# diharaw/hybrid-rendering

Hardware: AMD Instinct MI355X
Metric: shadow Mrays/s over the fully denoised frame (1 spp trace + SVGF temporal + 4x a-trous) (higher is better)
Workload: dtype f32; 1 GPU; 1920x1080 procedural Sponza-like (277968 tris) ray-traced shadows 1spp + SVGF denoise; trace_launch_order=heaviest tiles of the last frame first (csrc/tile_order.h), rays_per_frame_per_gpu=729543, pixels_per_gpu=2073600, bvh_nodes=23425

## Files before the change

hybrid_rendering_amd/api.py:

```python
from __future__ import annotations

import ctypes as C
import os

import numpy as np

_HERE = os.path.dirname(os.path.abspath(__file__))
LIB_PATH = os.environ.get("HR_LIBRARY") or os.path.join(_HERE, "libhybrid_rendering_amd.so")



class hr_light(C.Structure):
    _fields_ = [("data0", C.c_float * 4), ("data1", C.c_float * 4), ("data2", C.c_float * 4), ("data3", C.c_float * 4)]


class hr_ubo(C.Structure):
    _fields_ = [("view_inverse", C.c_float * 16), ("proj_inverse", C.c_float * 16), ("view_proj_inverse", C.c_float * 16),
                ("prev_view_proj", C.c_float * 16), ("view_proj", C.c_float * 16), ("cam_pos", C.c_float * 4),
                ("current_prev_jitter", C.c_float * 4), ("light", hr_light)]


assert C.sizeof(hr_ubo) == 416


# ... 28 lines not shown


class hr_band(C.Structure):
    _fields_ = [("band_y0", C.c_int32), ("band_y1", C.c_int32), ("halo", C.c_int32), ("history_halo", C.c_int32)]


HR_MAX_STAGES = 16


class hr_stage_times(C.Structure):
    _fields_ = [("n_stages", C.c_int32), ("name", C.c_char_p * HR_MAX_STAGES), ("ms", C.c_float * HR_MAX_STAGES), ("bytes", C.c_uint64 * HR_MAX_STAGES)]


class hr_shadows_params(C.Structure):
    _fields_ = [("denoise", C.c_int32), ("bias", C.c_float), ("alpha", C.c_float), ("moments_alpha", C.c_float), ("phi_visibility", C.c_float),
                ("phi_normal", C.c_float), ("sigma_depth", C.c_float), ("power", C.c_float), ("radius", C.c_int32),
                ("filter_iterations", C.c_int32), ("feedback_iteration", C.c_int32), ("exact", C.c_int32)]


class hr_ao_params(C.Structure):
    _fields_ = [("denoise", C.c_int32), ("ray_length", C.c_float), ("bias", C.c_float), ("alpha", C.c_float), ("blur_radius", C.c_int32),
                ("power", C.c_float), ("spp", C.c_int32), ("exact", C.c_int32)]


HR_FORMAT = {1: ("R32_UINT", 4), 2: ("R16F", 2), 3: ("RG16F", 4), 4: ("RGBA16F", 8), 5: ("R32F", 4), 6: ("RGBA8", 4), 0: ("R8", 1)}
OUTPUT_RAY_TRACE, OUTPUT_TEMPORAL_ACCUMULATION, OUTPUT_ATROUS, OUTPUT_UPSAMPLE = 0, 1, 2, 3
SCALE_FULL_RES, SCALE_HALF_RES, SCALE_QUARTER_RES = 0, 1, 2

ABI_SYMBOLS = [
    "hr_status_string", "hr_last_error", "hr_version", "hr_api_revision", "hr_ctx_create", "hr_ctx_destroy", "hr_ctx_device", "hr_scene_create", "hr_scene_get_info", "hr_scene_id", "hr_scene_create_instanced", "hr_scene_update_instances", "hr_scene_instance_count", "hr_scene_rebuild_top_level", "hr_scene_top_level_rebuilds", "hr_scene_read_bvh", "hr_set_markers", "hr_markers_log",
    "hr_scene_destroy", "hr_trace_any_hit", "hr_trace_closest_hit", "hr_gbuffer_raycast", "hr_shadows_default_params", "hr_shadows_create",
    "hr_shadows_render", "hr_shadows_output", "hr_shadows_reset_history", "hr_shadows_destroy", "hr_shadows_ray_trace", "hr_shadows_denoise", "hr_shadows_temporal",
    "hr_shadows_atrous_iteration", "hr_shadows_upsample", "hr_shadows_image", "hr_shadows_history_apron_exceeded", "hr_shadows_set_profiling", "hr_shadows_get_stage_times",
    "hr_gbuffer_mip_nearest", "hr_bvh_build_info", "hr_bvh_selfcheck", "hr_shadows_ray_count", "hr_shadows_tile_ray_counts", "hr_shadows_trace_stats", "hr_shadows_trace_stats_timed", "hr_shadows_launch_order", "hr_shadows_trace_divergence", "hr_selftest_math",
]

_lib = None


class HRError(RuntimeError):
    pass


def lib():
    global _lib
    if _lib is None:
        if not os.path.exists(LIB_PATH):
            raise HRError(f"{LIB_PATH} not built: run `python -m hybrid_rendering_amd.build` (hipcc, gfx950). No CPU fallback exists.")
        try:
            import torch
        except Exception:
            pass
        _lib = C.CDLL(LIB_PATH)
        _lib.hr_status_string.restype = C.c_char_p
        _lib.hr_last_error.restype = C.c_char_p
        _lib.hr_version.restype = C.c_char_p
        _lib.hr_scene_id.restype = C.c_uint64
        _lib.hr_scene_id.argtypes = [C.c_void_p]
    return _lib


def _check(status: int, what: str):
    if status != 0:
        L = lib()
        raise HRError(f"{what}: {L.hr_status_string(status).decode()} — {L.hr_last_error().decode()}")


# ... 368 lines not shown
```

hybrid_rendering_amd/csrc/device_math.h:

```cpp
#pragma once
#include <hip/hip_runtime.h>
#include <stdint.h>

#define HR_DEV __device__ __forceinline__

namespace hr {

struct f3 { float x, y, z; };

HR_DEV float hr_sqrt(float x) { return __builtin_sqrtf(x); }
HR_DEV f3 mk3(float x, float y, float z) { f3 r; r.x = x; r.y = y; r.z = z; return r; }
HR_DEV f3 add3(f3 a, f3 b) { return mk3(a.x + b.x, a.y + b.y, a.z + b.z); }
HR_DEV f3 sub3(f3 a, f3 b) { return mk3(a.x - b.x, a.y - b.y, a.z - b.z); }
HR_DEV f3 scale3(f3 a, float s) { return mk3(a.x * s, a.y * s, a.z * s); }
HR_DEV f3 neg3(f3 a) { return mk3(-a.x, -a.y, -a.z); }
HR_DEV float dot3(f3 a, f3 b) { return (a.x * b.x + a.y * b.y) + a.z * b.z; }
HR_DEV f3 cross3(f3 a, f3 b) { return mk3(a.y * b.z - b.y * a.z, a.z * b.x - b.z * a.x, a.x * b.y - b.x * a.y); }
HR_DEV float len3(f3 a) { return hr_sqrt(dot3(a, a)); }
HR_DEV f3 normalize3(f3 a)
{
    float inv = __fdiv_rn(1.0f, hr_sqrt(dot3(a, a)));
    return scale3(a, inv);
}
HR_DEV float min2(float a, float b) { return a < b ? a : b; }
// ... 65 lines not shown
};
HR_DEV DivBy div_prepare(float d)
{
    DivBy D;
    D.d = d;
    const float r0 = __builtin_amdgcn_rcpf(d);
    const float e0 = hr_fma(-d, r0, 1.0f);
    D.r1   = hr_fma(e0, r0, r0);
    D.fast = d >= 1e-6f && d <= 1e6f;
    return D;
}
HR_DEV float div_by(float n, const DivBy& D)
{
    const float an = fabsf(n);
    if (D.fast && (n == 0.0f || (an >= 1e-12f && an <= 3e5f)))
    {
        const float q0 = n * D.r1;
        const float e1 = hr_fma(-D.d, q0, n);
        const float q1 = hr_fma(e1, D.r1, q0);
        const float e2 = hr_fma(-D.d, q1, n);
        return hr_fma(e2, D.r1, q1);
    }
    return __fdiv_rn(n, D.d);
}
HR_DEV float div_by_inrange(float n, const DivBy& D)
{
    const float q0 = n * D.r1;
    const float e1 = hr_fma(-D.d, q0, n);
    const float q1 = hr_fma(e1, D.r1, q0);
    const float e2 = hr_fma(-D.d, q1, n);
    return hr_fma(e2, D.r1, q1);
}
HR_DEV float div_by_if(bool inrange, float n, const DivBy& D) { return inrange ? div_by_inrange(n, D) : __fdiv_rn(n, D.d); }

HR_DEV float det_log(float x)
{
    if (x <= 0.0f) return -1.0e30f;
    uint32_t u = __float_as_uint(x);
    int      e = (int)(u >> 23) - 126;
    float    m = __uint_as_float((u & 0x007fffffu) | 0x3f000000u);
    if (m < 0.707106781186547524f)
    {
        e -= 1;
        m = m + m - 1.0f;
    }
    else
        m = m - 1.0f;
    float z  = m * m;
    float y  = ((((((((7.0376836292e-2f * m - 1.1514610310e-1f) * m + 1.1676998740e-1f) * m - 1.2420140846e-1f) * m + 1.4249322787e-1f) * m - 1.6668057665e-1f) * m + 2.0000714765e-1f) * m - 2.4999993993e-1f) * m + 3.3333331174e-1f) * m * z;
    float fe = (float)e;
    y        = y + fe * -2.12194440e-4f;
    y        = y - 0.5f * z;
    float r  = m + y;
    r        = r + fe * 0.693359375f;
    return r;
}

HR_DEV float det_pow(float x, float y)
{
    if (x <= 0.0f) return 0.0f;
    return det_exp(y * det_log(x));
}

HR_DEV float det_powi(float x, int n)
{
    float r = 1.0f, b = x;
// ... 23 lines not shown
        float nx = (1.0f - fabsf(v.y)) * (step1(0.0f, v.x) * 2.0f - 1.0f);
        float ny = (1.0f - fabsf(v.x)) * (step1(0.0f, v.y) * 2.0f - 1.0f);
        v.x = nx;
        v.y = ny;
    }
    return normalize3(v);
}

HR_DEV void oct_encode(f3 n, float& ox, float& oy)
{
    float inv = __fdiv_rn(1.0f, (fabsf(n.x) + fabsf(n.y)) + fabsf(n.z));
    float px = n.x * inv, py = n.y * inv;
    if (n.z > 0.0f) { ox = px; oy = py; }
    else
    {
        ox = (1.0f - fabsf(py)) * (step1(0.0f, px) * 2.0f - 1.0f);
        oy = (1.0f - fabsf(px)) * (step1(0.0f, py) * 2.0f - 1.0f);
    }
}

HR_DEV int trace_lane_kind(int x, int y, int w, int h, int y0, int y1)
{
    const int gy = (y >> 2) << 2;
    if (gy >= h) return 0;
    if (y < h) return (y < y0 || y >= y1) ? 0 : (x < w ? 1 : 2);
    return (gy >= y0 && gy < y1) ? 2 : 0;
}

HR_DEV f3 world_pos_from_depth(float u, float v, float ndc_depth, const float* __restrict__ view_proj_inverse)
{
    f4 wp = mul_m4(view_proj_inverse, u * 2.0f - 1.0f, v * 2.0f - 1.0f, ndc_depth, 1.0f);
    return mk3(__fdiv_rn(wp.x, wp.w), __fdiv_rn(wp.y, wp.w), __fdiv_rn(wp.z, wp.w));
}

HR_DEV float luminance(f3 rgb) { return max2(dot3(rgb, mk3(0.299f, 0.587f, 0.114f)), 0.0001f); }

HR_DEV uint32_t blue_noise_texel(int cx, int cy, const uint8_t* __restrict__ sr) { return *(const uint32_t*)(sr + (((cy & 127) * 128 + (cx & 127)) << 2)); }
HR_DEV float sample_blue_noise_t(uint32_t t, int sample_index, int dim, const uint8_t* __restrict__ sobol)
{
    sample_index &= 255;
    dim &= 3;
    int ranked = sample_index ^ (int)((t >> 16) & 0xffu);
    int value  = (int)sobol[ranked * 4 + dim];
    value ^= (int)((t >> ((dim & 1) * 8)) & 0xffu);
    return (0.5f + (float)value) * 0.00390625f;
}
HR_DEV float sample_blue_noise(int cx, int cy, int sample_index, int dim, const uint8_t* __restrict__ sobol, const uint8_t* __restrict__ sr)
{
    return sample_blue_noise_t(blue_noise_texel(cx, cy, sr), sample_index, dim, sobol);
}

}
```

hybrid_rendering_amd/csrc/shading.h:

```cpp
#pragma once
#include "../../include/hr_api.h"
#include "traverse.h"

#ifdef HR_PROBE_FAST_HIT
namespace hr { HR_DEV f3 probe_normalize3(f3 a) { return scale3(a, __builtin_amdgcn_rsqf(dot3(a, a))); } }
#define __fdiv_rn(a, b) ((a) * __builtin_amdgcn_rcpf(b))
#define hr_sqrt(x) __builtin_amdgcn_sqrtf(x)
#define normalize3(v) probe_normalize3(v)
#endif

namespace hr {

#define HR_EPSILON 0.0001f

struct Rng { uint32_t x, y; };
HR_DEV uint32_t rng_rotl(uint32_t x, uint32_t k) { return (x << k) | (x >> (32 - k)); }
HR_DEV uint32_t rng_next(Rng& r)
{
    uint32_t result = r.x * 0x9e3779bbu;
    r.y ^= r.x;
    r.x = rng_rotl(r.x, 26) ^ r.y ^ (r.y << 9);
    r.y = rng_rotl(r.y, 13);
    return result;
}
// ... 475 lines not shown
            {
                const float* qt = s.tangents + q * 9;
                tg = add3(add3(scale3(mk3(qt[0], qt[1], qt[2]), b0), scale3(mk3(qt[3], qt[4], qt[5]), b1)), scale3(mk3(qt[6], qt[7], qt[8]), b2));
            }
            tg = ir ? normalize3(inst_mul3(ir->m, normalize3(tg))) : normalize3(normalize3(tg));
            const f3 T = normalize3(tg), Nn = normalize3(o.N);
            sample_texture(s, mt[1], tu, tv, c);
            const f3 tn = normalize3(sub3(scale3(mk3(c[0], c[1], c[2]), 2.0f), one3()));
            o.N = normalize3(add3(add3(scale3(T, tn.x), scale3(T, tn.y)), scale3(Nn, tn.z)));
        }
    }
    return o;
}

HR_DEV void fetch_light_hard(const hr_light& L, f3 Wo, f3 P, f3 N, f3& Li, f3& Wi, f3& Wh, float& t_max, float& attenuation)
{
    const int type = (int)L.data3[0];
    const f3  ldir = mk3(L.data0[0], L.data0[1], L.data0[2]);
    Li = scale3(mk3(L.data2[0], L.data2[1], L.data2[2]), L.data0[3]);
    if (type == 0) { Wi = ldir; t_max = 10000.0f; attenuation = 1.0f; }
    else
    {
        const f3 to_light = sub3(mk3(L.data1[0], L.data1[1], L.data1[2]), P);
        Wi                = normalize3(to_light);
        const float dist  = len3(to_light);
        t_max             = dist;
        if (type == 1) attenuation = __fdiv_rn(1.0f, dist * dist);
        else attenuation = __fdiv_rn(smoothstep1(L.data3[1], L.data3[2], dot3(Wi, ldir)), dist * dist);
    }
    Wh          = normalize3(add3(Wo, Wi));
    attenuation = attenuation * clamp1(dot3(N, Wi), 0.0f, 1.0f);
}

HR_DEV void fetch_light_shadow(const hr_light& L, f3 P, f3 N, float rx, float ry, f3& Wi, float& t_max, float& attenuation)
{
    const int type = (int)L.data3[0];
    const f3  ldir = mk3(L.data0[0], L.data0[1], L.data0[2]);
    f3        light_dir;
    float     radius;
    if (type == 0)
    {
        light_dir   = ldir;
        radius      = L.data1[3];
        t_max       = 10000.0f;
        attenuation = 1.0f;
    }
    else
    {
        f3    to_light = sub3(mk3(L.data1[0], L.data1[1], L.data1[2]), P);
        light_dir      = normalize3(to_light);
        float dist     = len3(to_light);
        radius         = __fdiv_rn(L.data1[3], dist);
        t_max          = dist;
        attenuation    = __fdiv_rn(1.0f, dist * dist);
    }
    f3    tangent   = normalize3(cross3(light_dir, mk3(0.0f, 1.0f, 0.0f)));
    f3    bitangent = normalize3(cross3(tangent, light_dir));
    float pr        = radius * hr_sqrt(rx);
    float pa        = ry * 2.0f * HR_M_PI;
    float s, c;
    det_sincos(pa, s, c);
    float dx = pr * c, dy = pr * s;
    Wi       = normalize3(add3(add3(light_dir, scale3(tangent, dx)), scale3(bitangent, dy)));
    if (type == 2)
    {
        float aa    = smoothstep1(L.data3[1], L.data3[2], dot3(Wi, ldir));
        attenuation = __fdiv_rn(aa, t_max * t_max);
    }
    attenuation = attenuation * clamp1(dot3(N, Wi), 0.0f, 1.0f);
}

struct TraceCtx
{
    const Node8*  nodes;
    const TriGPU* tris;
    uint32_t*     wave_stack;
    int           lane;
    DivCounters*  dv = nullptr;
    uint32_t      nn = 0, nt = 0;
};

template <bool STATS = false>
HR_DEV f3 direct_lighting(TraceCtx& tc, const hr_light& light, f3 Wo, f3 N, f3 P, f3 F0, f3 diffuse_color, float roughness, f3 T,
                          bool sample_sky, float r2x, float r2y, const CubeMap& sky, uint32_t& rays)
{
    f3       Lo = mk3(0.0f, 0.0f, 0.0f);
    const f3 ray_origin = add3(P, scale3(N, 0.1f));
    uint32_t nn = 0, nt = 0;
    {
        f3    Li, Wi, Wh;
        float t_max, attenuation;
        fetch_light_hard(light, Wo, P, N, Li, Wi, Wh, t_max, attenuation);
#ifndef HR_ABL_NO_SECONDARY
        if (attenuation > 0.0f)
        {
            rays++;
            attenuation = attenuation * (trace_any<STATS>(tc.nodes, tc.tris, ray_origin, Wi, 0.01f, t_max, tc.wave_stack, tc.lane, nn, nt, 0u, tc.dv) ? 0.0f : 1.0f);
        }
#endif
        const f3 brdf = evaluate_uber_brdf(diffuse_color, roughness, N, F0, Wo, Wh, Wi);
        Lo = add3(Lo, mul3(scale3(mul3(T, brdf), attenuation), Li));
    }
// ... 62 lines not shown
```

hybrid_rendering_amd/csrc/shadows.hip:

```cpp
#include "hr_internal.h"
#include "reproject.h"
#include "traverse.h"
#include "shading.h"
#include "upsample.h"
#include "pass_args.h"
#include "tile_order.h"

using namespace hr;

struct TraceArgs
{
    float           vpi[16];
    hr_light        light;
    const float*    depth;
    const uint2*    gb2;
    const uint8_t*  sobol;
    const uint8_t*  sr;
    uint32_t*       mask;
    uint16_t*       ray_slots;
    const Node8*    nodes;
    const TriGPU*   tris;
    unsigned long long* stats;
    unsigned long long* timeline;
    int             w, h;
    int             y0, y1;
    int             mw;
    int             tiles_x, tiles_y, tile_y0, debug_skip_traversal, debug_only_tx, debug_only_ty;
    float           bias;
    uint32_t        num_frames;
    uint32_t*       occluder;
    uint32_t        n_tri_refs;
    const uint32_t* order;
    uint16_t*       cost;
};

#define TRACE_WAVES 1
#ifndef SHADOWS_TRACE_EU
#define SHADOWS_TRACE_EU 1
#endif
template <bool STATS>
__global__ __launch_bounds__(64 * TRACE_WAVES, SHADOWS_TRACE_EU) void k_shadows_trace(TraceArgs a)
{
    __shared__ uint32_t s_stack[TRACE_WAVES][HR_STACK_ENTRIES * 64];
    const int lane = threadIdx.x & 63, wave = threadIdx.x >> 6;
    const int launch_slot = blockIdx.x * TRACE_WAVES + wave;
    if (launch_slot >= a.tiles_x * a.tiles_y) return;
    const int slot = a.order ? (int)a.order[launch_slot] : launch_slot;
    const int tx = slot % a.tiles_x, ty_local = slot / a.tiles_x, ty = ty_local + a.tile_y0;
    if (a.debug_only_tx >= 0 && (tx != a.debug_only_tx || ty != a.debug_only_ty)) return;
    unsigned long long t_begin = 0;
    if (a.timeline || a.cost) t_begin = wall_clock64();
    const int x = tx * 8 + (lane & 7), y = ty * 8 + (lane >> 3);
    bool      lit = false, fired = false;
    uint32_t  nn = 0, nt = 0, wave_max = 0;
    const int    kind = trace_lane_kind(x, y, a.w, a.h, a.y0, a.y1);
    const size_t pix  = kind == 1 ? (size_t)y * a.w + x : (size_t)a.y0 * a.w;
    const float    d_pre  = a.depth[pix];
    const uint2    g2_pre = a.gb2[pix];
    const uint32_t bn_pre = blue_noise_texel(x, y, a.sr);
    const uint32_t occ_pre = a.occluder ? a.occluder[pix] : 0xffffffffu;
    if (kind)
    {
        const float d = kind == 1 ? d_pre : 0.0f;
        if (d != 1.0f)
        {
            const float tu = __fdiv_rn((float)x + 0.5f, (float)a.w), tv = __fdiv_rn((float)y + 0.5f, (float)a.h);
            const f3    P  = world_pos_from_depth(tu, tv, d, a.vpi);
            const uint2 g2 = kind == 1 ? g2_pre : make_uint2(0u, 0u);
            const f3    N  = oct_decode(h2f_lo(g2.x), h2f_hi(g2.x));
            const f3    ro = add3(P, scale3(N, a.bias));
            const float r0 = sample_blue_noise_t(bn_pre, (int)a.num_frames, 0, a.sobol);
            const float r1 = sample_blue_noise_t(bn_pre, (int)a.num_frames, 1, a.sobol);
            f3    Wi;
            float t_max, att;
            fetch_light_shadow(a.light, P, N, r0, r1, Wi, t_max, att);
            if (att > 0.0f)
            {
                fired = true;
                bool occluded = false;
                uint32_t hit_tri = 0xffffffffu;
                if (a.occluder && kind == 1 && !a.debug_skip_traversal)
                {
                    const uint32_t c = occ_pre;
                    if (c < a.n_tri_refs)
                    {
                        const RayPre rp = ray_prepare(ro, Wi);
                        float t, u, v;
                        occluded = ray_tri_raw<false>(rp, load_tri_raw(a.tris, c), 0.01f, t_max, t, u, v);
                        if (STATS) nt++;
                        hit_tri = c;
                    }
                }
                if (a.debug_skip_traversal) lit = (ro.x + Wi.y > -1e30f);
                else if (!occluded)
                {
                    hit_tri = 0xffffffffu;
                    occluded = trace_any<STATS>(a.nodes, a.tris, ro, Wi, 0.01f, t_max, s_stack[wave], lane, nn, nt, 0u, nullptr, &hit_tri);
                }
                if (!a.debug_skip_traversal) lit = !occluded;
                if (a.occluder && kind == 1 && hit_tri != occ_pre) a.occluder[pix] = hit_tri;
            }
        }
    }
    const unsigned long long bits = __ballot(lit);
    const unsigned long long fb   = __ballot(fired);
    if (STATS)
    {
        uint32_t mx = nn + nt;
        for (int o = 32; o > 0; o >>= 1) { uint32_t t = __shfl_down(mx, o); mx = t > mx ? t : mx; }
        wave_max = mx;
        for (int o = 32; o > 0; o >>= 1) { nn += __shfl_down(nn, o); nt += __shfl_down(nt, o); }
    }
    if (lane == 0)
    {
        const int my = ty * 2;
        if (my * 4 >= a.y0 && my * 4 < a.y1) a.mask[(size_t)my * a.mw + tx] = (uint32_t)(bits & 0xffffffffull);
        if ((my + 1) * 4 >= a.y0 && (my + 1) * 4 < a.y1 && (my + 1) * 4 < a.h) a.mask[(size_t)(my + 1) * a.mw + tx] = (uint32_t)(bits >> 32);
        a.ray_slots[(size_t)ty * a.tiles_x + tx] = (uint16_t)__popcll(fb);
        if (a.cost)
        {
            const unsigned long long ticks = wall_clock64() - t_begin;
            a.cost[slot] = (uint16_t)(ticks > 65535ull ? 65535ull : ticks);
        }
        if (a.timeline)
        {
            const unsigned long long t_end = wall_clock64();
            uint32_t hw;
            asm volatile("s_getreg_b32 %0, hwreg(HW_REG_HW_ID)" : "=s"(hw));
            uint32_t xcc;
            asm volatile("s_getreg_b32 %0, hwreg(HW_REG_XCC_ID)" : "=s"(xcc));
// ... 349 lines not shown
    int     full_w = 0, full_h = 0, w = 0, h = 0, scale = 0;
    int     y0 = 0, y1 = 0;
    int     band_y0 = 0, band_y1 = 0;
    int     ry0 = 0, ry1 = 0;
    int     mw = 0, mh = 0, tiles_x = 0, tiles_y = 0;
    DevBuf  mask, temporal_out, moments[2], prev_image, atrous[2], upsample, tile_class, counters, nd, ray_slots, occluder;
    bool    occluder_cache = true;
    bool    first_frame = true;
    int     read_idx = 0;
    bool    last_denoise = true;
    int     last_ping_pong = 0;
    StageProfiler prof;
    hipStream_t   last_stream = nullptr;
    bool          want_stats = false;
    int           latched_exact = -1;
    bool          fuse = true;
    bool          persistent_waves = false;
    int           dbg_only_tx = -1, dbg_only_ty = -1;
    bool          dbg_skip_traversal = false, dbg_skip_reproject = false, dbg_timeline_stats = false;
    std::string   dbg_timeline;
    uint64_t      last_wave_max_steps = 0;
    bool          geo_history = true;
    bool          geo_valid = false;
    bool          dbg_require_geo = false;
    int           geo_parity = 0;
    const void*   geo_gb2 = nullptr;
    const void*   geo_gb3 = nullptr;
    void*         nd_cur = nullptr;
    TileOrder     tile_order;
};

bool hr::profiling_enabled(const hr_shadows* p) { return p && p->prof.enabled; }

extern "C" {

void hr_shadows_default_params(hr_shadows_params* p)
{
    p->denoise = 1; p->bias = 0.5f; p->alpha = 0.01f; p->moments_alpha = 0.2f; p->phi_visibility = 10.0f;
    p->phi_normal = 32.0f; p->sigma_depth = 1.0f; p->power = 1.2f; p->radius = 1; p->filter_iterations = 4; p->feedback_iteration = 1;
    p->exact = 1;
}

hr_status hr_shadows_create(hr_ctx* ctx, int32_t full_width, int32_t full_height, hr_scale scale, const hr_band* band, hr_shadows** out)
{
    HR_CHECK_ARG(ctx && out && full_width > 0 && full_height > 0 && (int)scale >= 0 && (int)scale <= 2);
    HR_HIP(hipSetDevice(ctx->device));
    hr_shadows* p = new hr_shadows();
    p->ctx = ctx; p->full_w = full_width; p->full_h = full_height; p->scale = (int)scale;
#ifdef HR_DEV_PATHS
    { const char* e = getenv("HR_TRACE_KERNEL"); p->persistent_waves = (e && std::string(e) == "queue"); }
#endif
    if (const char* e = getenv("HR_DEBUG_ONLY_TILE")) sscanf(e, "%d,%d", &p->dbg_only_tx, &p->dbg_only_ty);
    if (const char* e = getenv("HR_FUSE")) p->fuse = atoi(e) != 0;
    if (const char* e = getenv("HR_SHADOW_CACHE")) p->occluder_cache = atoi(e) != 0;
    if (const char* e = getenv("HR_GEO_HISTORY")) p->geo_history = atoi(e) != 0;
    if (const char* e = getenv("HR_DEBUG_REQUIRE_GEO")) p->dbg_require_geo = atoi(e) != 0;
    if (const char* e = getenv("HR_TILE_ORDER")) p->tile_order.enabled = atoi(e) != 0;
    p->tile_order.tag = "shadows";
    p->tile_order.min_spread = HR_ORDER_COHERENT_SPREAD;
    p->dbg_skip_traversal = getenv("HR_DEBUG_SKIP_TRAVERSAL") != nullptr;
    p->dbg_skip_reproject = getenv("HR_DEBUG_SKIP_REPROJECT") != nullptr;
    p->dbg_timeline_stats = getenv("HR_DEBUG_TIMELINE_STATS") != nullptr;
    if (const char* e = getenv("HR_DEBUG_TIMELINE")) p->dbg_timeline = e;
    p->w = full_width >> (int)scale; p->h = full_height >> (int)scale;
    p->y0 = 0; p->y1 = p->h; p->band_y0 = 0; p->band_y1 = p->h; p->ry0 = 0; p->ry1 = p->h;
    if (band && band->band_y1 > band->band_y0)
    {
// ... 106 lines not shown
}

hr_status hr_shadows_launch_order(hr_shadows* p, uint32_t* out, int32_t* n_tiles)
{
    HR_CHECK_ARG(p);
    return p->tile_order.read(out, n_tiles, p->last_stream);
}

static hr_status check_inputs(const hr_shadows* p, const hr_frame_inputs* in, bool need_prev)
{
    HR_CHECK_ARG(in->cur.depth && in->cur.gb2 && in->cur.gb3);
    HR_CHECK_ARG(in->cur.width == p->w && in->cur.height == p->h);
    if (need_prev) HR_CHECK_ARG(in->prev.depth && in->prev.gb2 && in->prev.gb3 && in->prev.width == p->w && in->prev.height == p->h);
    return HR_OK;
}

hr_status hr_shadows_ray_trace(hr_shadows* p, const hr_scene* scene, const hr_frame_inputs* in, const hr_shadows_params* prm, void* stream_)
{
    HR_CHECK_ARG(p && scene && in && prm);
    hr_status s = check_inputs(p, in, false);
    if (s != HR_OK) return s;
    HR_CHECK_ARG(in->sobol && in->scrambling_ranking);
    hipStream_t st = (hipStream_t)stream_;
    p->last_stream = st;
    if (p->first_frame)
    {
        HR_HIP(hipMemsetAsync(p->prev_image.p, 0, p->prev_image.bytes, st));
        HR_HIP(hipMemsetAsync(p->moments[!in->ping_pong].p, 0, p->moments[0].bytes, st));
        p->first_frame = false;
    }
    TraceArgs a;
    for (int i = 0; i < 16; i++) a.vpi[i] = in->ubo.view_proj_inverse[i];
    a.light = in->ubo.light;
    a.depth = in->cur.depth; a.gb2 = (const uint2*)in->cur.gb2;
    a.sobol = in->sobol; a.sr = in->scrambling_ranking;
    a.mask = (uint32_t*)p->mask.p; a.ray_slots = (uint16_t*)p->ray_slots.p;
    a.nodes = (const Node8*)scene->nodes.p; a.tris = (const TriGPU*)scene->tris.p;
    a.stats = nullptr;
    a.timeline = nullptr;
    a.w = p->w; a.h = p->h; a.y0 = p->y0; a.y1 = p->y1; a.mw = p->mw;
    a.tile_y0 = p->y0 / 8; a.tiles_x = p->tiles_x; a.tiles_y = cdiv(p->y1, 8) - a.tile_y0;
    a.bias = prm->bias; a.num_frames = in->num_frames;
    a.occluder = p->occluder_cache ? (uint32_t*)p->occluder.p : nullptr;
    a.n_tri_refs = (uint32_t)(scene->tris.bytes / sizeof(TriGPU));
    const int n_tiles = a.tiles_x * a.tiles_y;
    const int n_slots = n_tiles;
    a.debug_only_tx = p->dbg_only_tx; a.debug_only_ty = p->dbg_only_ty;
    a.debug_skip_traversal = p->dbg_skip_traversal ? 1 : 0;
    if ((s = p->tile_order.flush(st)) != HR_OK) return s;
    a.order = p->tile_order.order_arg(n_tiles); a.cost = p->tile_order.cost_arg(n_tiles);
    const uint64_t px = (uint64_t)p->w * (p->y1 - p->y0);
    if (p->want_stats)
    {
        a.cost = nullptr;
        HR_HIP(hipMemsetAsync((char*)p->counters.p + 16, 0, 24, st));
        a.stats = (unsigned long long*)((char*)p->counters.p + 16);
#ifdef HR_DEV_PATHS
        if (p->persistent_waves) hipLaunchKernelGGL(k_shadows_trace_pw<true>, dim3(cdiv(n_tiles, PW_TILES)), dim3(256), 0, st, a);
        else
#endif
        hipLaunchKernelGGL(k_shadows_trace<true>, dim3(cdiv(n_slots, TRACE_WAVES)), dim3(64 * TRACE_WAVES), 0, st, a);
        HR_HIP(hipGetLastError());
        return HR_OK;
    }
    if (!p->dbg_timeline.empty())
    {
// ... 289 lines not shown
```

hybrid_rendering_amd/csrc/traverse.h:

```cpp
#pragma once
#include "bvh.h"
#include "device_math.h"

namespace hr {

#define HR_STACK_ENTRIES 16
#define HR_SPILL_ENTRIES 48
static_assert(HR_STACK_ENTRIES + HR_SPILL_ENTRIES >= hr::kMaxTraversalDepth, "traversal stack shallower than the deepest BVH hr_scene_create accepts");

struct DivCounters { uint32_t lane_nodes, lane_pairs, wave_nodes, wave_pairs; };
#ifdef HR_TRACE_DIVERGENCE
#define HR_DIV(...) __VA_ARGS__
HR_DEV void div_count(uint32_t& lane_ctr, uint32_t& wave_ctr)
{
    lane_ctr++;
    const unsigned long long b = __ballot(1);
    if ((int)(threadIdx.x & 63) == __ffsll((long long)b) - 1) wave_ctr++;
}
HR_DEV void div_flush(const DivCounters& c, unsigned long long* g)
{
    uint32_t ln = c.lane_nodes, lp = c.lane_pairs, wn = c.wave_nodes, wp = c.wave_pairs, mn = c.lane_nodes, mp = c.lane_pairs, act = c.lane_nodes ? 1u : 0u;
    for (int o = 32; o > 0; o >>= 1)
    {
        ln += __shfl_xor(ln, o); lp += __shfl_xor(lp, o); wn += __shfl_xor(wn, o); wp += __shfl_xor(wp, o); act += __shfl_xor(act, o);
// ... 17 lines not shown
    float Sx, Sy, Sz;
    float idx, idy, idz;
    float ox, oy, oz;
    uint32_t sel;
};

HR_DEV float pick(f3 v, int k) { return k == 0 ? v.x : (k == 1 ? v.y : v.z); }

HR_DEV RayPre ray_prepare(f3 o, f3 d)
{
    RayPre r;
    r.o = o;
    float ax = fabsf(d.x), ay = fabsf(d.y), az = fabsf(d.z);
    int   kz = 0;
    if (ay > ax) kz = 1;
    if (az > (kz == 0 ? ax : ay)) kz = 2;
    int kx = kz + 1; if (kx == 3) kx = 0;
    int ky = kx + 1; if (ky == 3) ky = 0;
    if (pick(d, kz) < 0.0f) { int t = kx; kx = ky; ky = t; }
    r.kx = kx; r.ky = ky; r.kz = kz;
    float dz = pick(d, kz);
    r.Sx = __fdiv_rn(pick(d, kx), dz);
    r.Sy = __fdiv_rn(pick(d, ky), dz);
    r.Sz = __fdiv_rn(1.0f, dz);
    const float tiny = 1e-18f;
    float dx_ = fabsf(d.x) < tiny ? (d.x < 0.0f ? -tiny : tiny) : d.x;
    float dy_ = fabsf(d.y) < tiny ? (d.y < 0.0f ? -tiny : tiny) : d.y;
    float dz_ = fabsf(d.z) < tiny ? (d.z < 0.0f ? -tiny : tiny) : d.z;
    r.idx = __builtin_amdgcn_rcpf(dx_); r.idy = __builtin_amdgcn_rcpf(dy_); r.idz = __builtin_amdgcn_rcpf(dz_);
    r.sel = (dx_ < 0.0f ? 1u : 0u) | (dy_ < 0.0f ? 2u : 0u) | (dz_ < 0.0f ? 4u : 0u);
    return r;
}

template <bool WANT_TUV>
HR_DEV bool ray_tri_perm(const RayPre& r, const int kx, const int ky, const int kz, f3 v0, f3 v1, f3 v2, float t_min, float t_max, float& t_out, float& u_out, float& v_out)
{
    f3 A = sub3(v0, r.o), B = sub3(v1, r.o), C = sub3(v2, r.o);
    float Akz = pick(A, kz), Bkz = pick(B, kz), Ckz = pick(C, kz);
    float Ax = pick(A, kx) - r.Sx * Akz, Ay = pick(A, ky) - r.Sy * Akz;
    float Bx = pick(B, kx) - r.Sx * Bkz, By = pick(B, ky) - r.Sy * Bkz;
    float Cx = pick(C, kx) - r.Sx * Ckz, Cy = pick(C, ky) - r.Sy * Ckz;
    float U = Cx * By - Cy * Bx;
    float V = Ax * Cy - Ay * Cx;
    float W = Bx * Ay - By * Ax;
    if ((U < 0.0f || V < 0.0f || W < 0.0f) && (U > 0.0f || V > 0.0f || W > 0.0f)) return false;
    float det = (U + V) + W;
    if (det == 0.0f) return false;
    float Az = r.Sz * Akz, Bz = r.Sz * Bkz, Cz = r.Sz * Ckz;
    float T  = (U * Az + V * Bz) + W * Cz;
    float sg = det < 0.0f ? -1.0f : 1.0f;
    float Ts = T * sg, ad = det * sg;
    if (!(Ts > t_min * ad && Ts < t_max * ad)) return false;
    if (WANT_TUV)
    {
        float inv = __fdiv_rn(1.0f, det);
        t_out = T * inv;
        u_out = V * inv;
        v_out = W * inv;
    }
    return true;
}
template <bool WANT_TUV>
HR_DEV bool ray_tri(const RayPre& r, f3 v0, f3 v1, f3 v2, float t_min, float t_max, float& t_out, float& u_out, float& v_out)
{
    return ray_tri_perm<WANT_TUV>(r, r.kx, r.ky, r.kz, v0, v1, v2, t_min, t_max, t_out, u_out, v_out);
}
// ... 174 lines not shown

#define HR_NO_ENTRY 0xffffffffu
HR_DEV uint32_t entry_node_for_box(const Node8* __restrict__ nodes, f3 lo, f3 hi)
{
    uint32_t ni = 0;
    for (int depth = 0; depth < 24; depth++)
    {
        const NodeRaw n = load_node(nodes, ni);
        const float nox = __uint_as_float(n.q0.x), noy = __uint_as_float(n.q0.y), noz = __uint_as_float(n.q0.z);
        const float sx = __uint_as_float((n.q0.w & 0xffu) << 23), sy = __uint_as_float(((n.q0.w >> 8) & 0xffu) << 23), sz = __uint_as_float(((n.q0.w >> 16) & 0xffu) << 23);
        const uint32_t wlo[6] = { n.q2.x, n.q2.y, n.q2.z, n.q2.w, n.q3.x, n.q3.y };
        const uint32_t whi[6] = { n.q3.z, n.q3.w, n.q4.x, n.q4.y, n.q4.z, n.q4.w };
        uint32_t ov = 0;
#pragma unroll
        for (int half = 0; half < 2; half++)
#pragma unroll
            for (int k = 0; k < 4; k++)
            {
                const bool o = hr_fma(ubyte(wlo[0 + half], k), sx, nox) <= hi.x && hr_fma(ubyte(whi[0 + half], k), sx, nox) >= lo.x &&
                               hr_fma(ubyte(wlo[2 + half], k), sy, noy) <= hi.y && hr_fma(ubyte(whi[2 + half], k), sy, noy) >= lo.y &&
                               hr_fma(ubyte(wlo[4 + half], k), sz, noz) <= hi.z && hr_fma(ubyte(whi[4 + half], k), sz, noz) >= lo.z;
                ov |= o ? (1u << (half * 4 + k)) : 0u;
            }
        ov &= (1u << (n.q0.w >> 28)) - 1u;
        if (ov == 0u) return HR_NO_ENTRY;
        const uint32_t imask = (1u << ((n.q0.w >> 24) & 15u)) - 1u;
        if ((ov & (ov - 1u)) != 0u || (ov & ~imask) != 0u) break;
        ni = n.q1.x + (uint32_t)__builtin_ctz(ov);
    }
    return ni;
}

template <bool STATS, int ORDER = HR_ANY_ORDER>
HR_DEV bool trace_any(const Node8* __restrict__ nodes, const TriGPU* __restrict__ tris, f3 o, f3 d, float t_min, float t_max,
                      uint32_t* wave_stack, int lane, uint32_t& n_nodes, uint32_t& n_tris, uint32_t entry = 0u, DivCounters* dv = nullptr,
                      uint32_t* hit_tri = nullptr)
{
    if (entry == HR_NO_ENTRY) return false;
    RayPre    r = ray_prepare(o, d);
    uint32_t  spill_array[HR_SPILL_ENTRIES];
    LaneStack st;
    st.init(wave_stack, lane, spill_array);
    uint32_t cur = (entry << 9) | 1u, ni;
    bool     hit = false;
    const int pcode = wave_perm_code(r);
    while (walk_next<ORDER != HR_ORDER_SLOTS>(cur, st, ni))
    {
        const NodeHits h = test_node<ORDER>(load_node(nodes, ni), r, t_min, t_max);
        if (STATS) n_nodes++;
        HR_DIV(if (dv) div_count(dv->lane_nodes, dv->wave_nodes);)
        uint32_t trimask = walk_expand(h, cur, st);
        while (trimask)
        {
            HR_DIV(if (dv) div_count(dv->lane_pairs, dv->wave_pairs);)
            const uint32_t i0 = (uint32_t)__builtin_ctz(trimask);
            trimask &= trimask - 1u;
            const bool     two = trimask != 0u;
            const uint32_t i1  = two ? (uint32_t)__builtin_ctz(trimask) : i0;
            trimask &= trimask - 1u;
            const TriRaw ta = load_tri_raw(tris, h.tri_base + i0), tb = load_tri_raw(tris, h.tri_base + i1);
            if (STATS) n_tris += two ? 2u : 1u;
            float t, u, v;
            const bool ha = ray_tri_raw_uniform<false>(r, pcode, ta, t_min, t_max, t, u, v);
            const bool hb = ray_tri_raw_uniform<false>(r, pcode, tb, t_min, t_max, t, u, v);
            if (ha || hb) { hit = true; if (hit_tri) *hit_tri = h.tri_base + (ha ? i0 : i1); break; }
        }
        if (hit) break;
    }
    return hit;
}


HR_DEV void     wave_fence() { __builtin_amdgcn_fence(__ATOMIC_SEQ_CST, "wavefront"); __builtin_amdgcn_wave_barrier(); }
HR_DEV uint32_t lanes_below(unsigned long long m) { return __builtin_amdgcn_mbcnt_hi((uint32_t)(m >> 32), __builtin_amdgcn_mbcnt_lo((uint32_t)m, 0u)); }

#ifdef HR_DEV_PATHS
struct RaySeq { float Sx, Sy, Sz, idx, idy, idz, t_max; uint32_t code; };

HR_DEV RaySeq rayseq_pack(const RayPre& r, float t_max)
{
    RaySeq q;
    q.t_max = t_max;
    q.Sx = r.Sx; q.Sy = r.Sy; q.Sz = r.Sz; q.idx = r.idx; q.idy = r.idy; q.idz = r.idz;
    q.code = (uint32_t)r.kx | ((uint32_t)r.ky << 2) | ((uint32_t)r.kz << 4) | (r.sel << 6);
    return q;
}
HR_DEV void rayseq_unpack(RayPre& r, const RaySeq& q)
{
    r.Sx = q.Sx; r.Sy = q.Sy; r.Sz = q.Sz; r.idx = q.idx; r.idy = q.idy; r.idz = q.idz;
    r.kx = (int)(q.code & 3u); r.ky = (int)((q.code >> 2) & 3u); r.kz = (int)((q.code >> 4) & 3u); r.sel = q.code >> 6;
}
template <int NB>
HR_DEV RaySeq rayseq_select(const RaySeq (&q)[NB], int s)
{
    RaySeq o = q[0];
#pragma unroll
    for (int k = 1; k < NB; k++)
        if (s == k) o = q[k];
    return o;
}

template <int NB, int ORDER = HR_ANY_ORDER>
// ... 291 lines not shown
```

include/hr_api_stages.h:

```cpp
#ifndef HR_API_STAGES_H
#define HR_API_STAGES_H
#ifndef HR_API_H
#error "include hr_api.h"
#endif
#ifdef __cplusplus
extern "C" {
#endif

hr_status hr_set_markers(int32_t mode);
int32_t   hr_markers_log(char* out, int32_t capacity);

hr_status hr_scene_read_bvh(const hr_scene* scene, void* nodes_out, void* tris_out);

hr_status hr_shadows_ray_trace(hr_shadows* p, const hr_scene* scene, const hr_frame_inputs* in, const hr_shadows_params* params, void* stream);
hr_status hr_shadows_denoise(hr_shadows* p, const hr_frame_inputs* in, const hr_shadows_params* params, void* stream);
hr_status hr_shadows_temporal(hr_shadows* p, const hr_frame_inputs* in, const hr_shadows_params* params, void* stream);
hr_status hr_shadows_atrous_iteration(hr_shadows* p, const hr_frame_inputs* in, const hr_shadows_params* params, int32_t iteration, void* stream);
hr_status hr_shadows_upsample(hr_shadows* p, const hr_frame_inputs* in, const hr_shadows_params* params, void* stream);
hr_status hr_shadows_image(hr_shadows* p, int32_t which, hr_image_view* view);
hr_status hr_shadows_history_apron_exceeded(hr_shadows* p, int32_t* exceeded);
hr_status hr_shadows_set_profiling(hr_shadows* p, int32_t enable);
hr_status hr_shadows_get_stage_times(hr_shadows* p, hr_stage_times* out);
hr_status hr_shadows_ray_count(hr_shadows* p, uint64_t* rays);
hr_status hr_shadows_tile_ray_counts(hr_shadows* p, uint16_t* out, int32_t* tiles_x, int32_t* tiles_y);
hr_status hr_shadows_trace_stats(hr_shadows* p, const hr_scene* scene, const hr_frame_inputs* in, const hr_shadows_params* params, uint64_t* out3, void* stream);
hr_status hr_shadows_launch_order(hr_shadows* p, uint32_t* out, int32_t* n_tiles);
hr_status hr_shadows_trace_stats_timed(hr_shadows* p, const hr_scene* scene, const hr_frame_inputs* in, const hr_shadows_params* params, uint64_t* out3, void* stream);
hr_status hr_shadows_trace_divergence(hr_shadows* p, uint64_t* wave_max_steps);

hr_status hr_ao_ray_trace(hr_ao* p, const hr_scene* scene, const hr_frame_inputs* in, const hr_ao_params* params, void* stream);
hr_status hr_ao_denoise(hr_ao* p, const hr_frame_inputs* in, const hr_ao_params* params, void* stream);
hr_status hr_ao_temporal(hr_ao* p, const hr_frame_inputs* in, const hr_ao_params* params, void* stream);
hr_status hr_ao_blur(hr_ao* p, const hr_frame_inputs* in, const hr_ao_params* params, int32_t pass, void* stream);
hr_status hr_ao_upsample(hr_ao* p, const hr_frame_inputs* in, const hr_ao_params* params, void* stream);
hr_status hr_ao_image(hr_ao* p, int32_t which, hr_image_view* view);
hr_status hr_ao_history_apron_exceeded(hr_ao* p, int32_t* exceeded);
hr_status hr_ao_set_profiling(hr_ao* p, int32_t enable);
hr_status hr_ao_get_stage_times(hr_ao* p, hr_stage_times* out);
hr_status hr_ao_ray_count(hr_ao* p, uint64_t* rays);
hr_status hr_ao_trace_stats(hr_ao* p, const hr_scene* scene, const hr_frame_inputs* in, const hr_ao_params* params, uint64_t* out3, void* stream);
hr_status hr_ao_launch_order(hr_ao* p, uint32_t* out, int32_t* n_tiles);

hr_status hr_ddgi_set_shard(hr_ddgi* p, int32_t probe_z0, int32_t probe_z1, int32_t row_y0, int32_t row_y1);
hr_status hr_ddgi_current_write(hr_ddgi* p, hr_image_view* irradiance, hr_image_view* depth);

hr_status hr_ddgi_ray_trace(hr_ddgi* p, const hr_scene* scene, const hr_frame_inputs* in, const hr_environment* env, const hr_ddgi_params* params, void* stream);
hr_status hr_ddgi_trace_stats(hr_ddgi* p, const hr_scene* scene, const hr_frame_inputs* in, const hr_environment* env, const hr_ddgi_params* params, uint64_t* out3, void* stream);
hr_status hr_ddgi_probe_update(hr_ddgi* p, void* stream);
hr_status hr_ddgi_sample_probe_grid(hr_ddgi* p, const hr_frame_inputs* in, const hr_ddgi_params* params, void* stream);
hr_status hr_ddgi_end_frame(hr_ddgi* p);
hr_status hr_ddgi_image(hr_ddgi* p, int32_t which, hr_image_view* view);
hr_status hr_ddgi_get_uniforms(hr_ddgi* p, hr_ddgi_uniforms* out);
hr_status hr_ddgi_set_profiling(hr_ddgi* p, int32_t enable);
hr_status hr_ddgi_get_stage_times(hr_ddgi* p, hr_stage_times* out);
hr_status hr_ddgi_ray_count(hr_ddgi* p, uint64_t* rays);

hr_status hr_reflections_ray_trace(hr_reflections* p, const hr_scene* scene, const hr_frame_inputs* in, const hr_environment* env, hr_ddgi* ddgi,
                                   const hr_reflections_params* params, void* stream);
hr_status hr_reflections_trace_stats(hr_reflections* p, const hr_scene* scene, const hr_frame_inputs* in, const hr_environment* env, hr_ddgi* ddgi,
                                     const hr_reflections_params* params, uint64_t* out3, void* stream);
hr_status hr_reflections_denoise(hr_reflections* p, const hr_frame_inputs* in, const hr_reflections_params* params, void* stream);
// ... 40 lines not shown
```

Measured before the change: 4602 Mrays/s.

## Hoist sun light frame to host and specialize ray setup per wave permutation

For directional lights, the light tangent frame is computed once on the host and passed in, so the trace kernel no longer builds it per ray. The divisions for pixel UV and world position are replaced by reciprocal-based division when inputs are in range, and correctly rounded division is kept as the fallback. Ray setup is specialized at compile time when every lane in a wave shares the same axis permutation, and the prepared ray is passed into trace_any instead of being rebuilt there. This cuts per-ray ALU work in the trace kernel, at the cost of more code paths and possible bitwise drift if the host and device frames differ.

```diff
diff --git a/hybrid_rendering_amd/api.py b/hybrid_rendering_amd/api.py
--- a/hybrid_rendering_amd/api.py
+++ b/hybrid_rendering_amd/api.py
@@ -84,7 +84,7 @@
     "hr_scene_destroy", "hr_trace_any_hit", "hr_trace_closest_hit", "hr_gbuffer_raycast", "hr_shadows_default_params", "hr_shadows_create",
     "hr_shadows_render", "hr_shadows_output", "hr_shadows_reset_history", "hr_shadows_destroy", "hr_shadows_ray_trace", "hr_shadows_denoise", "hr_shadows_temporal",
     "hr_shadows_atrous_iteration", "hr_shadows_upsample", "hr_shadows_image", "hr_shadows_history_apron_exceeded", "hr_shadows_set_profiling", "hr_shadows_get_stage_times",
-    "hr_gbuffer_mip_nearest", "hr_bvh_build_info", "hr_bvh_selfcheck", "hr_shadows_ray_count", "hr_shadows_tile_ray_counts", "hr_shadows_trace_stats", "hr_shadows_trace_stats_timed", "hr_shadows_launch_order", "hr_shadows_trace_divergence", "hr_selftest_math",
+    "hr_gbuffer_mip_nearest", "hr_bvh_build_info", "hr_bvh_selfcheck", "hr_shadows_ray_count", "hr_shadows_tile_ray_counts", "hr_shadows_trace_stats", "hr_shadows_trace_stats_timed", "hr_shadows_launch_order", "hr_shadows_trace_divergence", "hr_shadows_sun_frame", "hr_selftest_math",
 ]
 
 _lib = None
diff --git a/hybrid_rendering_amd/csrc/device_math.h b/hybrid_rendering_amd/csrc/device_math.h
--- a/hybrid_rendering_amd/csrc/device_math.h
+++ b/hybrid_rendering_amd/csrc/device_math.h
@@ -121,6 +121,8 @@
     return hr_fma(e2, D.r1, q1);
 }
 HR_DEV float div_by_if(bool inrange, float n, const DivBy& D) { return inrange ? div_by_inrange(n, D) : __fdiv_rn(n, D.d); }
+HR_DEV float div_by_signed(float n, const DivBy& D, float d) { return __builtin_amdgcn_div_fixupf(div_by_inrange(n, D), d, n); }
+HR_DEV bool div_num_inrange(float n) { const float an = fabsf(n); return (an == 0.0f) | ((an >= 1e-12f) & (an <= 3e5f)); }
 
 HR_DEV float det_log(float x)
 {
@@ -210,6 +212,15 @@
     f4 wp = mul_m4(view_proj_inverse, u * 2.0f - 1.0f, v * 2.0f - 1.0f, ndc_depth, 1.0f);
     return mk3(__fdiv_rn(wp.x, wp.w), __fdiv_rn(wp.y, wp.w), __fdiv_rn(wp.z, wp.w));
 }
+HR_DEV f3 world_pos_from_depth_shared(float u, float v, float ndc_depth, const float* __restrict__ view_proj_inverse)
+{
+    f4 wp = mul_m4(view_proj_inverse, u * 2.0f - 1.0f, v * 2.0f - 1.0f, ndc_depth, 1.0f);
+    const DivBy D  = div_prepare(fabsf(wp.w));
+    const bool  nx = div_num_inrange(wp.x), ny = div_num_inrange(wp.y), nz = div_num_inrange(wp.z);
+    const bool  ok = D.fast & nx & ny & nz;
+    if (__any(!ok)) return mk3(__fdiv_rn(wp.x, wp.w), __fdiv_rn(wp.y, wp.w), __fdiv_rn(wp.z, wp.w));
+    return mk3(div_by_signed(wp.x, D, wp.w), div_by_signed(wp.y, D, wp.w), div_by_signed(wp.z, D, wp.w));
+}
 
 HR_DEV float luminance(f3 rgb) { return max2(dot3(rgb, mk3(0.299f, 0.587f, 0.114f)), 0.0001f); }
 
diff --git a/hybrid_rendering_amd/csrc/shading.h b/hybrid_rendering_amd/csrc/shading.h
--- a/hybrid_rendering_amd/csrc/shading.h
+++ b/hybrid_rendering_amd/csrc/shading.h
@@ -531,6 +531,25 @@
     attenuation = attenuation * clamp1(dot3(N, Wi), 0.0f, 1.0f);
 }
 
+struct LightFrame { f3 dir, tangent, bitangent; };
+HR_DEV LightFrame light_frame(f3 light_dir)
+{
+    LightFrame F;
+    F.dir       = light_dir;
+    F.tangent   = normalize3(cross3(light_dir, mk3(0.0f, 1.0f, 0.0f)));
+    F.bitangent = normalize3(cross3(F.tangent, light_dir));
+    return F;
+}
+HR_DEV f3 light_disc_dir(const LightFrame& F, float radius, float rx, float ry)
+{
+    float pr = radius * hr_sqrt(rx);
+    float pa = ry * 2.0f * HR_M_PI;
+    float s, c;
+    det_sincos(pa, s, c);
+    float dx = pr * c, dy = pr * s;
+    return normalize3(add3(add3(F.dir, scale3(F.tangent, dx)), scale3(F.bitangent, dy)));
+}
+
 HR_DEV void fetch_light_shadow(const hr_light& L, f3 P, f3 N, float rx, float ry, f3& Wi, float& t_max, float& attenuation)
 {
     const int type = (int)L.data3[0];
@@ -553,20 +572,21 @@
         t_max          = dist;
         attenuation    = __fdiv_rn(1.0f, dist * dist);
     }
-    f3    tangent   = normalize3(cross3(light_dir, mk3(0.0f, 1.0f, 0.0f)));
-    f3    bitangent = normalize3(cross3(tangent, light_dir));
-    float pr        = radius * hr_sqrt(rx);
-    float pa        = ry * 2.0f * HR_M_PI;
-    float s, c;
-    det_sincos(pa, s, c);
-    float dx = pr * c, dy = pr * s;
-    Wi       = normalize3(add3(add3(light_dir, scale3(tangent, dx)), scale3(bitangent, dy)));
+    const LightFrame F = light_frame(light_dir);
+    Wi                 = light_disc_dir(F, radius, rx, ry);
     if (type == 2)
     {
         float aa    = smoothstep1(L.data3[1], L.data3[2], dot3(Wi, ldir));
         attenuation = __fdiv_rn(aa, t_max * t_max);
     }
     attenuation = attenuation * clamp1(dot3(N, Wi), 0.0f, 1.0f);
+}
+
+HR_DEV void fetch_sun_shadow(const LightFrame& F, float radius, f3 N, float rx, float ry, f3& Wi, float& t_max, float& attenuation)
+{
+    t_max       = 10000.0f;
+    Wi          = light_disc_dir(F, radius, rx, ry);
+    attenuation = 1.0f * clamp1(dot3(N, Wi), 0.0f, 1.0f);
 }
 
 struct TraceCtx
diff --git a/hybrid_rendering_amd/csrc/shadows.hip b/hybrid_rendering_amd/csrc/shadows.hip
--- a/hybrid_rendering_amd/csrc/shadows.hip
+++ b/hybrid_rendering_amd/csrc/shadows.hip
@@ -32,6 +32,8 @@
     uint32_t        n_tri_refs;
     const uint32_t* order;
     uint16_t*       cost;
+    LightFrame      sun;
+    int             use_sun;
 };
 
 #define TRACE_WAVES 1
@@ -59,13 +61,17 @@
     const uint2    g2_pre = a.gb2[pix];
     const uint32_t bn_pre = blue_noise_texel(x, y, a.sr);
     const uint32_t occ_pre = a.occluder ? a.occluder[pix] : 0xffffffffu;
+    const bool  uv_shared = a.w >= 1 && a.w <= 262144 && a.h >= 1 && a.h <= 262144;
+    const DivBy Dw = div_prepare((float)a.w), Dh = div_prepare((float)a.h);
     if (kind)
     {
         const float d = kind == 1 ? d_pre : 0.0f;
         if (d != 1.0f)
         {
-            const float tu = __fdiv_rn((float)x + 0.5f, (float)a.w), tv = __fdiv_rn((float)y + 0.5f, (float)a.h);
-            const f3    P  = world_pos_from_depth(tu, tv, d, a.vpi);
+            float tu, tv;
+            if (uv_shared) { tu = div_by_inrange((float)x + 0.5f, Dw); tv = div_by_inrange((float)y + 0.5f, Dh); }
+            else { tu = __fdiv_rn((float)x + 0.5f, (float)a.w); tv = __fdiv_rn((float)y + 0.5f, (float)a.h); }
+            const f3    P  = world_pos_from_depth_shared(tu, tv, d, a.vpi);
             const uint2 g2 = kind == 1 ? g2_pre : make_uint2(0u, 0u);
             const f3    N  = oct_decode(h2f_lo(g2.x), h2f_hi(g2.x));
             const f3    ro = add3(P, scale3(N, a.bias));
@@ -73,10 +79,13 @@
             const float r1 = sample_blue_noise_t(bn_pre, (int)a.num_frames, 1, a.sobol);
             f3    Wi;
             float t_max, att;
-            fetch_light_shadow(a.light, P, N, r0, r1, Wi, t_max, att);
+            if (a.use_sun) fetch_sun_shadow(a.sun, a.light.data1[3], N, r0, r1, Wi, t_max, att);
+            else fetch_light_shadow(a.light, P, N, r0, r1, Wi, t_max, att);
             if (att > 0.0f)
             {
                 fired = true;
+                const int    pcode = dir_wave_perm_code(Wi);
+                const RayPre rp    = ray_prepare_uniform(ro, Wi, pcode);
                 bool occluded = false;
                 uint32_t hit_tri = 0xffffffffu;
                 if (a.occluder && kind == 1 && !a.debug_skip_traversal)
@@ -84,9 +93,8 @@
                     const uint32_t c = occ_pre;
                     if (c < a.n_tri_refs)
                     {
-                        const RayPre rp = ray_prepare(ro, Wi);
                         float t, u, v;
-                        occluded = ray_tri_raw<false>(rp, load_tri_raw(a.tris, c), 0.01f, t_max, t, u, v);
+                        occluded = ray_tri_raw_uniform<false>(rp, pcode, load_tri_raw(a.tris, c), 0.01f, t_max, t, u, v);
                         if (STATS) nt++;
                         hit_tri = c;
                     }
@@ -95,7 +103,7 @@
                 else if (!occluded)
                 {
                     hit_tri = 0xffffffffu;
-                    occluded = trace_any<STATS>(a.nodes, a.tris, ro, Wi, 0.01f, t_max, s_stack[wave], lane, nn, nt, 0u, nullptr, &hit_tri);
+                    occluded = trace_any<STATS>(a.nodes, a.tris, rp, pcode, 0.01f, t_max, s_stack[wave], lane, nn, nt, 0u, nullptr, &hit_tri);
                 }
                 if (!a.debug_skip_traversal) lit = !occluded;
                 if (a.occluder && kind == 1 && hit_tri != occ_pre) a.occluder[pix] = hit_tri;
@@ -511,7 +519,35 @@
 
 bool hr::profiling_enabled(const hr_shadows* p) { return p && p->prof.enabled; }
 
+static float sun_nan_canonical(float v)
+{
+    return v != v ? __builtin_bit_cast(float, 0x7fc00000u) : v;
+}
+static f3 sun_cross(f3 a, f3 b) { return f3{ a.y * b.z - b.y * a.z, a.z * b.x - b.z * a.x, a.x * b.y - b.x * a.y }; }
+static f3 sun_normalize(f3 a)
+{
+    const float inv = 1.0f / sqrtf((a.x * a.x + a.y * a.y) + a.z * a.z);
+    return f3{ sun_nan_canonical(a.x * inv), sun_nan_canonical(a.y * inv), sun_nan_canonical(a.z * inv) };
+}
+static LightFrame sun_frame(const hr_light& L)
+{
+    LightFrame F;
+    F.dir       = f3{ L.data0[0], L.data0[1], L.data0[2] };
+    F.tangent   = sun_normalize(sun_cross(F.dir, f3{ 0.0f, 1.0f, 0.0f }));
+    F.bitangent = sun_normalize(sun_cross(F.tangent, F.dir));
+    return F;
+}
+
 extern "C" {
+
+hr_status hr_shadows_sun_frame(const hr_light* light, float* out9)
+{
+    HR_CHECK_ARG(light && out9);
+    const LightFrame F = sun_frame(*light);
+    const float v[9] = { F.dir.x, F.dir.y, F.dir.z, F.tangent.x, F.tangent.y, F.tangent.z, F.bitangent.x, F.bitangent.y, F.bitangent.z };
+    for (int i = 0; i < 9; i++) out9[i] = v[i];
+    return HR_OK;
+}
 
 void hr_shadows_default_params(hr_shadows_params* p)
 {
@@ -684,6 +720,8 @@
     TraceArgs a;
     for (int i = 0; i < 16; i++) a.vpi[i] = in->ubo.view_proj_inverse[i];
     a.light = in->ubo.light;
+    a.use_sun = a.light.data3[0] >= 0.0f && a.light.data3[0] < 1.0f ? 1 : 0;
+    a.sun     = sun_frame(a.light);
     a.depth = in->cur.depth; a.gb2 = (const uint2*)in->cur.gb2;
     a.sobol = in->sobol; a.sr = in->scrambling_ranking;
     a.mask = (uint32_t*)p->mask.p; a.ray_slots = (uint16_t*)p->ray_slots.p;
diff --git a/hybrid_rendering_amd/csrc/traverse.h b/hybrid_rendering_amd/csrc/traverse.h
--- a/hybrid_rendering_amd/csrc/traverse.h
+++ b/hybrid_rendering_amd/csrc/traverse.h
@@ -73,6 +73,64 @@
     return r;
 }
 
+HR_DEV int dir_perm_code(f3 d)
+{
+    const float ax = fabsf(d.x), ay = fabsf(d.y), az = fabsf(d.z);
+    int kz = 0;
+    if (ay > ax) kz = 1;
+    if (az > (kz == 0 ? ax : ay)) kz = 2;
+    return kz * 2 + (pick(d, kz) < 0.0f ? 1 : 0);
+}
+HR_DEV int dir_wave_perm_code(f3 d)
+{
+    const int c = dir_perm_code(d), c0 = __builtin_amdgcn_readfirstlane(c);
+    return __all(c == c0) ? c0 : -1;
+}
+
+template <int KX, int KY, int KZ>
+HR_DEV RayPre ray_prepare_perm(f3 o, f3 d)
+{
+    RayPre r;
+    r.o = o;
+    r.kx = KX; r.ky = KY; r.kz = KZ;
+    const float dz = pick(d, KZ), nx = pick(d, KX), ny = pick(d, KY);
+    const DivBy D  = div_prepare(fabsf(dz));
+    const bool  okx = div_num_inrange(nx), oky = div_num_inrange(ny);
+    const bool  ok  = D.fast & okx & oky;
+    if (__any(!ok))
+    {
+        r.Sx = __fdiv_rn(nx, dz);
+        r.Sy = __fdiv_rn(ny, dz);
+        r.Sz = __fdiv_rn(1.0f, dz);
+    }
+    else
+    {
+        r.Sx = div_by_signed(nx, D, dz);
+        r.Sy = div_by_signed(ny, D, dz);
+        r.Sz = div_by_signed(1.0f, D, dz);
+    }
+    const float tiny = 1e-18f;
+    float dx_ = fabsf(d.x) < tiny ? (d.x < 0.0f ? -tiny : tiny) : d.x;
+    float dy_ = fabsf(d.y) < tiny ? (d.y < 0.0f ? -tiny : tiny) : d.y;
+    float dz_ = fabsf(d.z) < tiny ? (d.z < 0.0f ? -tiny : tiny) : d.z;
+    r.idx = __builtin_amdgcn_rcpf(dx_); r.idy = __builtin_amdgcn_rcpf(dy_); r.idz = __builtin_amdgcn_rcpf(dz_);
+    r.sel = (dx_ < 0.0f ? 1u : 0u) | (dy_ < 0.0f ? 2u : 0u) | (dz_ < 0.0f ? 4u : 0u);
+    return r;
+}
+HR_DEV RayPre ray_prepare_uniform(f3 o, f3 d, int code)
+{
+    switch (code)
+    {
+    case 0: return ray_prepare_perm<1, 2, 0>(o, d);
+    case 1: return ray_prepare_perm<2, 1, 0>(o, d);
+    case 2: return ray_prepare_perm<2, 0, 1>(o, d);
+    case 3: return ray_prepare_perm<0, 2, 1>(o, d);
+    case 4: return ray_prepare_perm<0, 1, 2>(o, d);
+    case 5: return ray_prepare_perm<1, 0, 2>(o, d);
+    default: return ray_prepare(o, d);
+    }
+}
+
 template <bool WANT_TUV>
 HR_DEV bool ray_tri_perm(const RayPre& r, const int kx, const int ky, const int kz, f3 v0, f3 v1, f3 v2, float t_min, float t_max, float& t_out, float& u_out, float& v_out)
 {
@@ -313,18 +371,16 @@
 }
 
 template <bool STATS, int ORDER = HR_ANY_ORDER>
-HR_DEV bool trace_any(const Node8* __restrict__ nodes, const TriGPU* __restrict__ tris, f3 o, f3 d, float t_min, float t_max,
+HR_DEV bool trace_any(const Node8* __restrict__ nodes, const TriGPU* __restrict__ tris, const RayPre& r, int pcode, float t_min, float t_max,
                       uint32_t* wave_stack, int lane, uint32_t& n_nodes, uint32_t& n_tris, uint32_t entry = 0u, DivCounters* dv = nullptr,
                       uint32_t* hit_tri = nullptr)
 {
     if (entry == HR_NO_ENTRY) return false;
-    RayPre    r = ray_prepare(o, d);
     uint32_t  spill_array[HR_SPILL_ENTRIES];
     LaneStack st;
     st.init(wave_stack, lane, spill_array);
     uint32_t cur = (entry << 9) | 1u, ni;
     bool     hit = false;
-    const int pcode = wave_perm_code(r);
     while (walk_next<ORDER != HR_ORDER_SLOTS>(cur, st, ni))
     {
         const NodeHits h = test_node<ORDER>(load_node(nodes, ni), r, t_min, t_max);
@@ -349,6 +405,15 @@
         if (hit) break;
     }
     return hit;
+}
+template <bool STATS, int ORDER = HR_ANY_ORDER>
+HR_DEV bool trace_any(const Node8* __restrict__ nodes, const TriGPU* __restrict__ tris, f3 o, f3 d, float t_min, float t_max,
+                      uint32_t* wave_stack, int lane, uint32_t& n_nodes, uint32_t& n_tris, uint32_t entry = 0u, DivCounters* dv = nullptr,
+                      uint32_t* hit_tri = nullptr)
+{
+    if (entry == HR_NO_ENTRY) return false;
+    const RayPre r = ray_prepare(o, d);
+    return trace_any<STATS, ORDER>(nodes, tris, r, wave_perm_code(r), t_min, t_max, wave_stack, lane, n_nodes, n_tris, entry, dv, hit_tri);
 }
 
 
diff --git a/include/hr_api_stages.h b/include/hr_api_stages.h
--- a/include/hr_api_stages.h
+++ b/include/hr_api_stages.h
@@ -27,6 +27,7 @@
 hr_status hr_shadows_launch_order(hr_shadows* p, uint32_t* out, int32_t* n_tiles);
 hr_status hr_shadows_trace_stats_timed(hr_shadows* p, const hr_scene* scene, const hr_frame_inputs* in, const hr_shadows_params* params, uint64_t* out3, void* stream);
 hr_status hr_shadows_trace_divergence(hr_shadows* p, uint64_t* wave_max_steps);
+hr_status hr_shadows_sun_frame(const hr_light* light, float* out9);
 
 hr_status hr_ao_ray_trace(hr_ao* p, const hr_scene* scene, const hr_frame_inputs* in, const hr_ao_params* params, void* stream);
 hr_status hr_ao_denoise(hr_ao* p, const hr_frame_inputs* in, const hr_ao_params* params, void* stream);
```

After: 4607 Mrays/s (median of 6 runs). Within noise of the previous version (+0.1%).
